# volume-em/empanada

Hardware: AMD Instinct MI355X
Metric: Mvox/s end-to-end 3D panoptic inference (incl. consensus); PQ vs CPU ref (higher is better)
Workload: dtype f32

## Files before the change

empanada_amd/_hip.py:

```python
import ctypes
import os

import torch

_HERE = os.path.dirname(os.path.abspath(__file__))
LIB_PATH = os.path.join(_HERE, 'libemp_hip.so')

MAX_KS = 11
MAX_CLASSES = 16
MAX_CENTERS = 4096
CENTER_LIMIT = 65535


class HipError(RuntimeError):
    pass


_c = ctypes
_P = _c.c_void_p
_I = _c.c_int
_L = _c.c_int64
_F = _c.c_float
_U32 = _c.c_uint32

SIGNATURES = {
    'emp_version': (_I, []),
    'emp_last_error': (_c.c_char_p, []),
    'emp_device_count': (_I, []),
    'emp_bn_act_nhwc': (_I, [_P, _P, _P, _P, _I, _L, _I, _P, _L, _P]),
    'emp_dwconv_nhwc': (_I, [_P, _P, _P, _I, _I, _I, _I, _I, _P, _P]),
    'emp_upsample_bilinear': (_I, [_P, _I, _I, _I, _I, _P, _P, _I, _I, _P, _P]),
    'emp_conv_bn_act_proj_nhwc': (_I, [_P, _P, _P, _P, _I] + [_I] * 10 + [_P, _I, _P, _P, _L, _P]),
    'emp_conv_k_slab': (_I, [_L, _I, _I, _I]),
    'emp_conv_k_slab_cin': (_I, [_L, _I, _I, _I, _I]),
    'emp_conv_k_slab_geom': (_I, [_L, _I, _I, _I, _I, _I, _I, _I, _I]),
    'emp_conv1x1_ws_eligible': (_I, [_L, _I, _I, _I, _I, _I, _I, _I]),
    'emp_conv1x1_ws_kind_for': (_I, [_L, _I, _I, _I, _I, _I, _I, _I, _I]),
    'emp_conv1x1_ws_launches': (_L, [_I]),
    'emp_gconv_chunk': (_I, [_I]),
    'emp_gconv3x3_bn_act_nhwc': (_I, [_P, _L, _P, _P, _P, _I, _I, _I, _I, _I, _I, _I, _P, _L, _P]),
    'emp_conv_bn_act_nhwc': (_I, [_P, _P, _P, _P, _P, _L, _I] + [_I] * 10 + [_P, _L, _P]),
    'emp_conv_splitk_plan': (_I, [_L, _I, _I, _I, _I]),
    'emp_conv_splitk_bn_act_nhwc': (_I, [_P, _P, _P, _P, _P, _L, _I] + [_I] * 11 + [_P, _P, _L, _P]),
    'emp_wino_input_transform': (_I, [_P, _I, _I, _I, _I, _I, _P, _L, _P, _P]),
    'emp_gemm_nt_batched': (_I, [_P, _P, _I, _L, _I, _I, _P, _P]),
    'emp_wino4_input_transform': (_I, [_P, _I, _I, _I, _I, _I, _P, _L, _P, _P]),
    'emp_wino4_output_transform': (_I, [_P, _P, _L, _I, _I, _I, _I, _I, _P, _P, _I, _P, _L, _P]),
    'emp_wino4_conv_bn_act_nhwc': (_I, [_P, _I, _I, _I, _I, _I, _P, _L, _P, _I, _P, _P, _I, _P, _L, _P]),
    'emp_wino4_fused_eligible': (_I, [_L, _I, _I, _I]),
    'emp_wino3_input_transform': (_I, [_P, _I, _I, _I, _I, _I, _P, _L, _P, _P]),
    'emp_wino3_output_transform': (_I, [_P, _P, _L, _I, _I, _I, _I, _I, _P, _P, _I, _P, _L, _P]),
    'emp_wino_gemm_fused': (_I, [_P, _I, _I, _I, _I, _I, _P, _L, _P, _I, _P, _P]),
    'emp_wino_output_transform': (_I, [_P, _P, _L, _I, _I, _I, _I, _I, _P, _P, _I, _P, _L, _P]),
    'emp_chain_class': (_I, [_L, _P, _P, _P, _I, _P, _P, _P, _P, _L, _L, _c.c_double, _c.c_double, _P, _P, _P, _P]),
    'emp_lsap_maximize': (_L, [_P, _L, _L, _P, _P]),
    'emp_slices_to_input': (_I, [_P, _L, _L, _L, _I, _I, _I, _I, _I, _F, _F, _P, _P]),
    'emp_slices_to_input_scaled': (_I, [_P, _L, _L, _L] + [_I] * 7 + [_P, _P, _P, _P, _I, _F, _F, _P, _P]),
    'emp_pointwise_out_nhwc': (_I, [_P, _P, _P, _L, _L, _I, _I, _P, _P]),
    'emp_bn_relu_maxpool_nhwc': (_I, [_P, _P, _P, _I, _I, _I, _I, _P, _P]),
    'emp_stem_conv7_bn_relu_maxpool': (_I, [_P, _P, _P, _P, _I, _I, _I, _P, _P]),
    'emp_logits_to_prob': (_I, [_P, _I, _I, _L, _P, _P]),
    'emp_upsample_bilinear_prob': (_I, [_P, _I, _I, _I, _I, _P, _P, _I, _I, _P, _I, _P]),
    'emp_pr_upsample2x': (_I, [_P, _I, _I, _I, _I, _P, _P, _P]),
    'emp_pr_topk_work_bytes': (_L, [_I, _L]),
    'emp_pr_topk': (_I, [_P, _I, _L, _I, _P, _L, _P, _P]),
    'emp_pr_point_sample': (_I, [_P, _L, _P, _I, _I, _I, _I, _I, _P, _I, _I, _I, _P, _P, _I, _P]),
    'emp_pr_scatter': (_I, [_P, _I, _P, _I, _I, _I, _L, _P, _P]),
    'emp_median_harden_stack': (_I, [_P, _I, _I, _L, _I, _F, _P, _P, _P]),
# ... 979 lines not shown
```

empanada_amd/csrc/emp_conv.hip:

```cpp
#include "emp_common.h"
#include "emp_wino4.h"
#include <stdlib.h>

typedef float f32x16 __attribute__((ext_vector_type(16)));

#define CG_BM 128
#define CG_BK 32
#define CG_THREADS 256

struct ConvGeom {
    const float *x, *w, *scale, *shift, *res;
    float *out;
    int N, H, W, Cin, OH, OW, Cout, KH, KW, stride, pad, dil, relu;
    int64_t M, out_ps, res_ps;
    int tiles_m, tiles_n;
    int64_t x_bs, w_bs, out_bs;
    const int32_t *tiles;
    const float *proj_w;
    float *proj_out;
    int proj_n;
    int64_t hw;
};

__device__ __attribute__((aligned(16))) float cg_zero_page[64];

__device__ __forceinline__ void cg_glds16(const float *src, unsigned lds_byte_addr)
{
    asm volatile("s_mov_b32 m0, %1\n\ts_nop 0\n\tglobal_load_lds_dwordx4 %0, off" ::"v"(src), "s"(lds_byte_addr) : "memory", "m0");
}

template <int N>
__device__ __forceinline__ void cg_wait_vm()
{
    asm volatile("s_waitcnt vmcnt(%0)" ::"n"(N) : "memory");
}

template <int NT, int MODE, bool RESPF = false, int BK = 32, bool PROJ = false, bool GLDS = false, bool GATE = false>
__global__ __launch_bounds__(CG_THREADS, (BK == 16 ? 3 : 2)) void conv_igemm_f32_kernel(ConvGeom g)
{
    constexpr int BN = 64 * NT;
    constexpr int CG_LD = GLDS ? BK : BK + 4;
    constexpr int NBUF = GLDS ? (BK == 16 ? 3 : 2) : 2;
    constexpr int TPR = BK / 4;
    constexpr int RPP = CG_THREADS / TPR;
    constexpr int AR = CG_BM / RPP;
    constexpr int BROWS = BN / RPP;
    constexpr int NF4 = BK / 8;
    constexpr int CLD = BN + 4;
    constexpr int A_ELEMS = NBUF * CG_BM * CG_LD, B_ELEMS = NBUF * BN * CG_LD;
    constexpr int EPI_ROWS = (A_ELEMS + B_ELEMS >= CG_BM * CLD) ? CG_BM : 64;
    constexpr int C_ELEMS = EPI_ROWS * CLD;
    constexpr int SMEM = (A_ELEMS + B_ELEMS) > C_ELEMS ? (A_ELEMS + B_ELEMS) : C_ELEMS;
    static_assert(MODE == 0 || BK == 32, "the fused Winograd loader is written for BK = 32");
    static_assert(!GLDS || MODE == 0, "LDS-direct staging: plain convolution / GEMM loader only");
    __shared__ __attribute__((aligned(16))) float smem[SMEM];
    float *As = smem, *Bs = smem + A_ELEMS;
    g.x += (int64_t)blockIdx.y * g.x_bs;
    g.w += (int64_t)blockIdx.y * g.w_bs;
    g.out += (int64_t)blockIdx.y * g.out_bs;

    const int T = g.tiles_m * g.tiles_n;
    const int chunk = (T + 7) >> 3;
    const int tile = (blockIdx.x & 7) * chunk + (blockIdx.x >> 3);
    if (tile >= T) return;
    const int tm = tile / g.tiles_n, tn = tile % g.tiles_n;
    const int64_t m0 = (int64_t)tm * CG_BM;
    const int n0 = tn * BN;

    const int tid = threadIdx.x;
    const int lrow = tid / TPR, lcol = (tid % TPR) * 4;

    int a_n[AR], a_iy[AR], a_ix[AR];
    bool a_ok[AR], b_ok[BROWS];
    const float *b_ptr[BROWS];
    const int taps = g.KH * g.KW;
    int w_off[4][4];
    unsigned w_mask[4];
    float w_su = 1.f, w_sv = 1.f;
    if constexpr (MODE == 0) {
#pragma unroll
        for (int i = 0; i < AR; ++i) {
            const int64_t p = m0 + lrow + RPP * i;
            a_ok[i] = p < g.M;
            const int64_t pp = a_ok[i] ? p : 0;
            const int ox = (int)(pp % g.OW);
            const int oy = (int)((pp / g.OW) % g.OH);
            a_n[i] = (int)(pp / ((int64_t)g.OW * g.OH));
// ... 133 lines not shown
        for (int it = 0; it < NRE; ++it) {
            const int64_t p = m0 + crow + it * RPI;
            rpre[it] = make_float4(0.f, 0.f, 0.f, 0.f);
            if (p < g.M && co + 3 < g.Cout) rpre[it] = *reinterpret_cast<const float4 *>(g.res + p * g.res_ps + co);
        }
    }

    if constexpr (GLDS) {
        constexpr int RPW = 64 / TPR;
        constexpr int NL = AR + BROWS;
        const int swz_ld = (BK == 16) ? ((lrow >> 2) & 3) : ((lrow >> 1) & 7);
        const int csw = (((tid % TPR) ^ swz_ld) * 4);
        const float *ga[AR], *gb[BROWS];
        bool ga_ok[AR];
        auto set_tap_g = [&](int tap) {
            const int ky = tap / g.KW, kx = tap - ky * g.KW;
#pragma unroll
            for (int i = 0; i < AR; ++i) {
                const int iy = a_iy[i] + ky * g.dil, ix = a_ix[i] + kx * g.dil;
                ga_ok[i] = a_ok[i] && iy >= 0 && iy < g.H && ix >= 0 && ix < g.W;
                ga[i] = ga_ok[i] ? g.x + (((int64_t)a_n[i] * g.H + iy) * g.W + ix) * g.Cin + csw : cg_zero_page + csw;
            }
        };
#pragma unroll
        for (int i = 0; i < BROWS; ++i) {
            const int cob = n0 + lrow + RPP * i;
            gb[i] = (cob < g.Cout) ? g.w + (int64_t)cob * taps * g.Cin + csw : cg_zero_page + csw;
        }
        set_tap_g(tap0);
        const unsigned lds0 = (unsigned)(size_t)(__attribute__((address_space(3))) float *)smem;
        const unsigned a_dst = __builtin_amdgcn_readfirstlane(lds0 + (unsigned)(RPW * wave * BK * 4));
        const unsigned b_dst = __builtin_amdgcn_readfirstlane(lds0 + (unsigned)((A_ELEMS + RPW * wave * BK) * 4));
        int gl_tap = tap0, gl_c0 = c00;
        auto issue_slab = [&](int ring) {
#pragma unroll
            for (int i = 0; i < AR; ++i)
                cg_glds16(ga[i] + (ga_ok[i] ? gl_c0 : 0), a_dst + (unsigned)((ring * CG_BM + RPP * i) * BK * 4));
#pragma unroll
            for (int i = 0; i < BROWS; ++i) {
                const bool ok = n0 + lrow + RPP * i < g.Cout;
                cg_glds16(gb[i] + (ok ? (int64_t)gl_tap * g.Cin + gl_c0 : 0), b_dst + (unsigned)((ring * BN + RPP * i) * BK * 4));
            }
            gl_c0 += BK;
            if (gl_c0 == g.Cin) {
                gl_c0 = 0;
                ++gl_tap;
                if (gl_tap < taps) set_tap_g(gl_tap);
            }
        };
        const int swz_rd = (BK == 16) ? ((r >> 2) & 3) : ((r >> 1) & 7);
        issue_slab(0);
        if (NBUF == 3 && S > 1) issue_slab(1);
        if (NBUF == 3 && S > 1) cg_wait_vm<NL>(); else cg_wait_vm<0>();
        __builtin_amdgcn_s_barrier();
        for (int s = 0; s < S; ++s) {
            const int ring = s % NBUF;
            if (s + NBUF - 1 < S) issue_slab((s + NBUF - 1) % NBUF);
            const float *Ar = &As[ring * CG_BM * CG_LD + (wm * 64 + r) * CG_LD];
            const float *Br = &Bs[ring * BN * CG_LD + (wn * 32 * NT + r) * CG_LD];
#pragma unroll
            for (int f = 0; f < NF4; ++f) {
                const int pc = (((hh * NF4 + f) ^ swz_rd) * 4);
                float4 fa[2], fb[NT];
#pragma unroll
                for (int i = 0; i < 2; ++i) fa[i] = *reinterpret_cast<const float4 *>(Ar + i * 32 * CG_LD + pc);
#pragma unroll
                for (int j = 0; j < NT; ++j) fb[j] = *reinterpret_cast<const float4 *>(Br + j * 32 * CG_LD + pc);
#pragma unroll
                for (int e = 0; e < 4; ++e) {
                    float av[2], bv[NT];
#pragma unroll
                    for (int i = 0; i < 2; ++i) av[i] = e == 0 ? fa[i].x : e == 1 ? fa[i].y : e == 2 ? fa[i].z : fa[i].w;
#pragma unroll
                    for (int j = 0; j < NT; ++j) bv[j] = e == 0 ? fb[j].x : e == 1 ? fb[j].y : e == 2 ? fb[j].z : fb[j].w;
#pragma unroll
                    for (int i = 0; i < 2; ++i)
#pragma unroll
                        for (int j = 0; j < NT; ++j)
                            acc[i][j] = __builtin_amdgcn_mfma_f32_32x32x2f32(av[i], bv[j], acc[i][j], 0, 0, 0);
                }
            }
            if (NBUF == 3 && s + 2 < S) cg_wait_vm<NL>(); else cg_wait_vm<0>();
            __builtin_amdgcn_s_barrier();
        }
    } else {
        CG_LOAD_NEXT();
        store_slab(0);
        if (S > 1) CG_LOAD_NEXT();
        __syncthreads();
        for (int s = 0; s < S; ++s) {
            const int buf = s & 1;
            const float *Ab = &As[buf * CG_BM * CG_LD + (wm * 64 + r) * CG_LD + hh * (BK / 2)];
            const float *Bb = &Bs[buf * BN * CG_LD + (wn * 32 * NT + r) * CG_LD + hh * (BK / 2)];
    #pragma unroll
            for (int half = 0; half < NF4 / 2; ++half) {
                float4 fa[2][2], fb[NT][2];
    #pragma unroll
                for (int q = 0; q < 2; ++q) {
    #pragma unroll
                    for (int i = 0; i < 2; ++i)
                        fa[i][q] = *reinterpret_cast<const float4 *>(Ab + i * 32 * CG_LD + half * 8 + q * 4);
    #pragma unroll
                    for (int j = 0; j < NT; ++j)
                        fb[j][q] = *reinterpret_cast<const float4 *>(Bb + j * 32 * CG_LD + half * 8 + q * 4);
                }
    #pragma unroll
                for (int q = 0; q < 2; ++q) {
    #pragma unroll
                    for (int e = 0; e < 4; ++e) {
                        float av[2], bv[NT];
    #pragma unroll
                        for (int i = 0; i < 2; ++i)
                            av[i] = e == 0 ? fa[i][q].x : e == 1 ? fa[i][q].y : e == 2 ? fa[i][q].z : fa[i][q].w;
    #pragma unroll
                        for (int j = 0; j < NT; ++j)
// ... 106 lines not shown
            if constexpr (PROJ) {
                float ps[4] = {0.f, 0.f, 0.f, 0.f};
                if (valid && co + 3 < g.Cout) {
#pragma unroll
                    for (int q = 0; q < 4; ++q)
                        if (q < g.proj_n) {
                            const float4 wq = *reinterpret_cast<const float4 *>(g.proj_w + (int64_t)q * g.Cout + co);
                            ps[q] = __fadd_rn(__fadd_rn(__fadd_rn(__fmul_rn(v[0], wq.x), __fmul_rn(v[1], wq.y)),
                                                        __fmul_rn(v[2], wq.z)), __fmul_rn(v[3], wq.w));
                        }
                }
                *reinterpret_cast<float4 *>(&Cs[lrow_c * CLD + ccol]) = make_float4(ps[0], ps[1], ps[2], ps[3]);
            }
        }
        if constexpr (PROJ) {
            __syncthreads();
            for (int idx = tid; idx < EPI_ROWS * g.proj_n; idx += CG_THREADS) {
                const int row_l = idx / g.proj_n, q = idx - row_l * g.proj_n;
                const int64_t p = m0 + rd * EPI_ROWS + row_l;
                if (p < g.M) {
                    float t = Cs[row_l * CLD + q];
#pragma unroll 8
                    for (int j = 1; j < C4; ++j) t = __fadd_rn(t, Cs[row_l * CLD + 4 * j + q]);
                    const int64_t img = p / g.hw;
                    atomicAdd(g.proj_out + (img * g.proj_n + q) * g.hw + (p - img * g.hw), t);
                }
            }
        }
    }
}

struct CgPlan {
    bool narrow, respf, glds;
    int slab, tiles_m, tiles_n;
};

static CgPlan cg_plan(int64_t M, int Cout, int batch, bool has_res, bool res_vec_ok, bool may_split_n = true, int cin = 32)
{
    CgPlan p;
    const int64_t wide_blocks = emp_cdiv(M, CG_BM) * emp_cdiv(Cout, 128) * batch;
    p.narrow = Cout <= 64 || (Cout % 128 != 0 && Cout % 128 <= 64 && Cout < 512) || (may_split_n && wide_blocks < 256);
    p.tiles_m = (int)emp_cdiv(M, CG_BM);
    p.tiles_n = (int)emp_cdiv(Cout, p.narrow ? 64 : 128);
    static const char *fnarrow = getenv("EMP_CONV_NARROW");
    static const char *norespf = getenv("EMP_CONV_NO_RESPF");
    if (fnarrow && fnarrow[0] == '1') {
        p.narrow = true;
        p.tiles_n = (int)emp_cdiv(Cout, 64);
    }
    p.respf = has_res && res_vec_ok && Cout % (p.narrow ? 64 : 128) == 0 && !norespf;
    static const char *force = getenv("EMP_CONV_BK");
    const int64_t blocks = (int64_t)p.tiles_m * p.tiles_n * batch;
    p.slab = blocks > 512 ? 16 : 32;
    if (force && force[0] == '1') p.slab = 16;
    if (force && force[0] == '3') p.slab = 32;
    if (p.respf) p.slab = 32;
    if (cin % 32 != 0) {
        p.slab = 16;
        p.respf = false;
    }
    static const char *noglds = getenv("EMP_CONV_NO_GLDS");
    p.glds = !noglds;
    return p;
}

extern "C" int emp_conv_k_slab(int64_t M, int Cout, int batch, int has_residual)
{
    return cg_plan(M, Cout, batch, has_residual != 0, true).slab;
}

extern "C" int emp_conv_k_slab_cin(int64_t M, int Cout, int batch, int has_residual, int Cin)
{
    return cg_plan(M, Cout, batch, has_residual != 0, true, true, Cin).slab;
}

extern "C" __attribute__((visibility("hidden"))) int emp_conv1x1_ws_kind(int64_t M, int Cin, int Cout, int KH, int KW, int stride, int pad, int relu, int has_residual);
extern "C" __attribute__((visibility("hidden"))) int emp_conv1x1_ws_launch(int kind, const float *x, const float *w, const float *scale, const float *shift,
                                     const float *res, int64_t res_ps, int relu, int64_t M, int Cin, int Cout,
                                     float *out, int64_t out_ps, void *stream);
extern "C" __attribute__((visibility("hidden"))) int emp_gemm_ws_eligible(int batch, int64_t M, int N, int K, int slab);
extern "C" __attribute__((visibility("hidden"))) int emp_gemm_ws_launch(const float *A, const float *B, int batch, int64_t M, int N, int K, float *C,
                                                                        void *stream);

extern "C" int emp_conv_k_slab_geom(int64_t M, int Cout, int has_residual, int Cin, int KH, int KW, int stride, int pad,
                                    int relu)
{
    if (emp_conv1x1_ws_kind(M, Cin, Cout, KH, KW, stride, pad, relu, has_residual) == 1) return 64;
    return cg_plan(M, Cout, 1, has_residual != 0 && relu != 2, true, true, Cin).slab;
}

extern "C" int emp_conv_bn_act_nhwc(const float *x, const float *w_okkc, const float *scale, const float *shift,
                                    const float *residual, int64_t res_pixel_stride, int relu, int N, int H, int W,
                                    int Cin, int Cout, int KH, int KW, int stride, int pad, int dil, float *out,
                                    int64_t out_pixel_stride, void *stream)
{
// ... 12 lines not shown
                "conv: x and w must be 16-byte aligned");
    EMP_REQUIRE(out != x, "conv: output cannot alias the input");
    if (N == 0) return EMP_OK;
    ConvGeom g;
    g.x = x; g.w = w_okkc; g.scale = scale; g.shift = shift; g.res = residual; g.out = out;
    g.N = N; g.H = H; g.W = W; g.Cin = Cin; g.OH = OH; g.OW = OW; g.Cout = Cout; g.KH = KH; g.KW = KW;
    g.stride = stride; g.pad = pad; g.dil = dil; g.relu = relu;
    g.M = (int64_t)N * OH * OW; g.out_ps = out_pixel_stride; g.res_ps = res_pixel_stride;
    g.x_bs = g.w_bs = g.out_bs = 0; g.tiles = nullptr; g.proj_w = nullptr; g.proj_out = nullptr; g.proj_n = 0; g.hw = 1;
    const bool res_vec_ok = (res_pixel_stride & 3) == 0 && (reinterpret_cast<uintptr_t>(residual) & 15) == 0;
    const bool io_vec_ok = res_vec_ok && (out_pixel_stride & 3) == 0 && (reinterpret_cast<uintptr_t>(out) & 15) == 0 &&
                           (!scale || (reinterpret_cast<uintptr_t>(scale) & 15) == 0) &&
                           (!shift || (reinterpret_cast<uintptr_t>(shift) & 15) == 0);
    const int ws = io_vec_ok && scale && shift ? emp_conv1x1_ws_kind(g.M, Cin, Cout, KH, KW, stride, pad, relu, residual != nullptr) : 0;
    if (ws == 1)
        return emp_conv1x1_ws_launch(1, x, w_okkc, scale, shift, residual, res_pixel_stride, relu, g.M, Cin, Cout, out,
                                     out_pixel_stride, stream);
    const CgPlan pl = cg_plan(g.M, Cout, 1, residual != nullptr && relu != 2, res_vec_ok, true, Cin);
    if (ws == 2 && !residual && pl.slab == 16)
        return emp_conv1x1_ws_launch(2, x, w_okkc, scale, shift, nullptr, res_pixel_stride, relu, g.M, Cin, Cout, out,
                                     out_pixel_stride, stream);
    if (ws == 3 && residual && pl.respf && pl.slab == 32 &&
        res_pixel_stride < (1 << 24) && out_pixel_stride < (1 << 24))
        return emp_conv1x1_ws_launch(3, x, w_okkc, scale, shift, residual, res_pixel_stride, relu, g.M, Cin, Cout, out,
                                     out_pixel_stride, stream);
    const bool narrow = pl.narrow, respf = pl.respf, bk16 = pl.slab == 16;
    EMP_REQUIRE((int64_t)pl.tiles_m * pl.tiles_n < (1LL << 28), "conv: too many tiles");
    g.tiles_m = pl.tiles_m;
    g.tiles_n = pl.tiles_n;
    const int T = g.tiles_m * g.tiles_n;
    const int grid = 8 * ((T + 7) / 8);
#define CG_GO(NT_, RES_, BK_, GL_) hipLaunchKernelGGL((conv_igemm_f32_kernel<NT_, 0, RES_, BK_, false, GL_>), dim3(grid), dim3(CG_THREADS), 0, emp_stream(stream), g)
#define CG_GATE(NT_, BK_) hipLaunchKernelGGL((conv_igemm_f32_kernel<NT_, 0, false, BK_, false, true, true>), dim3(grid), dim3(CG_THREADS), 0, emp_stream(stream), g)
    if (relu == 2) {
        if (narrow) { if (bk16) CG_GATE(1, 16); else CG_GATE(1, 32); }
        else { if (bk16) CG_GATE(2, 16); else CG_GATE(2, 32); }
    } else if (narrow) {
        if (respf) { if (pl.glds) CG_GO(1, true, 32, true); else CG_GO(1, true, 32, false); }
        else if (pl.glds) { if (bk16) CG_GO(1, false, 16, true); else CG_GO(1, false, 32, true); }
        else { if (bk16) CG_GO(1, false, 16, false); else CG_GO(1, false, 32, false); }
    } else {
        if (respf) { if (pl.glds) CG_GO(2, true, 32, true); else CG_GO(2, true, 32, false); }
        else if (pl.glds) { if (bk16) CG_GO(2, false, 16, true); else CG_GO(2, false, 32, true); }
        else { if (bk16) CG_GO(2, false, 16, false); else CG_GO(2, false, 32, false); }
    }
#undef CG_GO
#undef CG_GATE
    EMP_CHECK_LAUNCH("emp_conv_bn_act_nhwc");
    return EMP_OK;
}

__global__ __launch_bounds__(256) void splitk_reduce_kernel(const float *__restrict__ work, int nz, int64_t M, int Cout,
                                                            const float *__restrict__ scale,
                                                            const float *__restrict__ shift,
                                                            const float *__restrict__ res, int64_t res_ps, int relu,
                                                            float *__restrict__ out, int64_t out_ps)
{
    const int C4 = Cout >> 2;
    const int64_t total = M * C4, plane = M * (int64_t)Cout;
    for (int64_t i = (int64_t)blockIdx.x * blockDim.x + threadIdx.x; i < total; i += (int64_t)gridDim.x * blockDim.x) {
        const int64_t p = i / C4;
        const int co = (int)(i - p * C4) * 4;
        const float *w = work + p * Cout + co;
        float4 t = *reinterpret_cast<const float4 *>(w);
        for (int z = 1; z < nz; ++z) {
            const float4 u = *reinterpret_cast<const float4 *>(w + z * plane);
            t.x = __fadd_rn(t.x, u.x); t.y = __fadd_rn(t.y, u.y); t.z = __fadd_rn(t.z, u.z); t.w = __fadd_rn(t.w, u.w);
        }
        float v[4] = {t.x, t.y, t.z, t.w};
#pragma unroll
        for (int e = 0; e < 4; ++e) {
            const float sc = scale ? scale[co + e] : 1.f, sh = shift ? shift[co + e] : 0.f;
            v[e] = __fadd_rn(__fmul_rn(v[e], sc), sh);
        }
        if (res) {
            const float4 r4 = *reinterpret_cast<const float4 *>(res + p * res_ps + co);
// ... 45 lines not shown
    EMP_REQUIRE(out != x && work != x && work != out, "conv_splitk: buffers must not alias");
    if (N == 0) return EMP_OK;
    ConvGeom g;
    g.x = x; g.w = w_okkc; g.scale = nullptr; g.shift = nullptr; g.res = nullptr; g.out = work;
    g.N = N; g.H = H; g.W = W; g.Cin = Cin; g.OH = OH; g.OW = OW; g.Cout = Cout; g.KH = KH; g.KW = KW;
    g.stride = stride; g.pad = pad; g.dil = dil; g.relu = 0;
    g.M = (int64_t)N * OH * OW; g.out_ps = Cout; g.res_ps = Cout;
    g.x_bs = g.w_bs = g.out_bs = 0; g.tiles = nullptr; g.proj_w = nullptr; g.proj_out = nullptr; g.proj_n = 0; g.hw = 1;
    const CgPlan pl = cg_plan(g.M, Cout, 1, false, true, true, Cin);
    EMP_REQUIRE((int64_t)pl.tiles_m * pl.tiles_n < (1LL << 28), "conv_splitk: too many tiles");
    g.tiles_m = pl.tiles_m;
    g.tiles_n = pl.tiles_n;
    const int T = g.tiles_m * g.tiles_n;
    const dim3 grid(8 * ((T + 7) / 8), 1, k_splits);
    hipStream_t st = emp_stream(stream);
    if (pl.narrow)
        hipLaunchKernelGGL((conv_igemm_f32_kernel<1, 0, false, 32, false, true>), grid, dim3(CG_THREADS), 0, st, g);
    else
        hipLaunchKernelGGL((conv_igemm_f32_kernel<2, 0, false, 32, false, true>), grid, dim3(CG_THREADS), 0, st, g);
    EMP_CHECK_LAUNCH("emp_conv_splitk_bn_act_nhwc(partials)");
    const int64_t total = g.M * (Cout / 4);
    hipLaunchKernelGGL(splitk_reduce_kernel, dim3(emp_grid(total, 256, 4096)), dim3(256), 0, st, work, k_splits, g.M, Cout,
                       scale, shift, residual, res_pixel_stride, relu, out, out_pixel_stride);
    EMP_CHECK_LAUNCH("emp_conv_splitk_bn_act_nhwc(reduce)");
    return EMP_OK;
}

extern "C" int emp_conv_bn_act_proj_nhwc(const float *x, const float *w_okkc, const float *scale, const float *shift,
                                         int relu, int N, int H, int W, int Cin, int Cout, int KH, int KW, int stride,
                                         int pad, int dil, const float *proj_w, int proj_n, float *proj_out,
                                         float *out, int64_t out_pixel_stride, void *stream)
{
    EMP_REQUIRE(x && w_okkc && proj_w && proj_out, "conv_proj: null pointer");
    EMP_REQUIRE(N >= 0 && H > 0 && W > 0 && Cin > 0 && Cin % CG_BK == 0, "conv_proj: bad shape (Cin %% %d)", CG_BK);
    EMP_REQUIRE(Cout == 128 || Cout == 256, "conv_proj: Cout %d must be 128 or 256 (at most two cout tiles)", Cout);
    EMP_REQUIRE(proj_n >= 1 && proj_n <= 4, "conv_proj: proj_n %d not in 1..4", proj_n);
    EMP_REQUIRE(KH >= 1 && KW >= 1 && KH <= 7 && KW <= 7 && stride >= 1 && dil >= 1 && pad >= 0, "conv_proj: bad filter geometry");
    const int OH = (H + 2 * pad - dil * (KH - 1) - 1) / stride + 1;
    const int OW = (W + 2 * pad - dil * (KW - 1) - 1) / stride + 1;
    EMP_REQUIRE(OH > 0 && OW > 0, "conv_proj: empty output");
    if (out_pixel_stride == 0) out_pixel_stride = Cout;
    EMP_REQUIRE(((reinterpret_cast<uintptr_t>(x) | reinterpret_cast<uintptr_t>(w_okkc) | reinterpret_cast<uintptr_t>(proj_w) |
                  reinterpret_cast<uintptr_t>(out)) & 15) == 0 && (out_pixel_stride & 3) == 0, "conv_proj: alignment");
    EMP_REQUIRE(out != x, "conv_proj: output cannot alias the input");
    if (N == 0) return EMP_OK;
    ConvGeom g;
    g.x = x; g.w = w_okkc; g.scale = scale; g.shift = shift; g.res = nullptr; g.out = out;
    g.N = N; g.H = H; g.W = W; g.Cin = Cin; g.OH = OH; g.OW = OW; g.Cout = Cout; g.KH = KH; g.KW = KW;
    g.stride = stride; g.pad = pad; g.dil = dil; g.relu = relu;
    g.M = (int64_t)N * OH * OW; g.out_ps = out_pixel_stride; g.res_ps = Cout;
    g.x_bs = g.w_bs = g.out_bs = 0; g.tiles = nullptr;
    g.proj_w = proj_w; g.proj_out = proj_out; g.proj_n = proj_n; g.hw = (int64_t)OH * OW;
    const CgPlan pl = cg_plan(g.M, Cout, 1, false, true, false);
    g.tiles_m = pl.tiles_m;
    g.tiles_n = pl.tiles_n;
    const int T = g.tiles_m * g.tiles_n;
    const int grid = 8 * ((T + 7) / 8);
#define CG_GOP(BK_, GL_) hipLaunchKernelGGL((conv_igemm_f32_kernel<2, 0, false, BK_, true, GL_>), dim3(grid), dim3(CG_THREADS), 0, emp_stream(stream), g)
    if (pl.glds) { if (pl.slab == 16) CG_GOP(16, true); else CG_GOP(32, true); }
    else { if (pl.slab == 16) CG_GOP(16, false); else CG_GOP(32, false); }
#undef CG_GOP
    EMP_CHECK_LAUNCH("emp_conv_bn_act_proj_nhwc");
    return EMP_OK;
}


__global__ __launch_bounds__(256) void wino_input_kernel(const float *__restrict__ x, const int32_t *__restrict__ tiles,
                                                         int64_t T, int H, int W, int C4, int dil, float4 *__restrict__ V)
{
    const int64_t total = T * C4;
    for (int64_t i = (int64_t)blockIdx.x * blockDim.x + threadIdx.x; i < total; i += (int64_t)gridDim.x * blockDim.x) {
        const int c4 = (int)(i % C4);
        const int64_t t = i / C4;
        const int n = tiles[3 * t], by = tiles[3 * t + 1], bx = tiles[3 * t + 2];
        const float4 *src = reinterpret_cast<const float4 *>(x) + (int64_t)n * H * W * C4 + c4;
        float4 d[4][4];
#pragma unroll
        for (int a = 0; a < 4; ++a)
#pragma unroll
            for (int b = 0; b < 4; ++b) {
                const int yy = by + a * dil, xx = bx + b * dil;
                d[a][b] = make_float4(0.f, 0.f, 0.f, 0.f);
                if (yy >= 0 && yy < H && xx >= 0 && xx < W) d[a][b] = src[((int64_t)yy * W + xx) * C4];
            }
#define W_SUB(p, q) make_float4(__fsub_rn(p.x, q.x), __fsub_rn(p.y, q.y), __fsub_rn(p.z, q.z), __fsub_rn(p.w, q.w))
#define W_ADD(p, q) make_float4(__fadd_rn(p.x, q.x), __fadd_rn(p.y, q.y), __fadd_rn(p.z, q.z), __fadd_rn(p.w, q.w))
        float4 tt[4][4];
#pragma unroll
        for (int a = 0; a < 4; ++a) {
            tt[a][0] = W_SUB(d[a][0], d[a][2]);
            tt[a][1] = W_ADD(d[a][1], d[a][2]);
            tt[a][2] = W_SUB(d[a][2], d[a][1]);
// ... 46 lines not shown
            for (int b = 0; b < 2; ++b) {
                const int yy = oy + a * dil, xx = ox + b * dil;
                if (yy < H && xx < W) {
                    float4 v = yv[b];
                    if (scale) v = make_float4(__fmul_rn(v.x, sc.x), __fmul_rn(v.y, sc.y), __fmul_rn(v.z, sc.z), __fmul_rn(v.w, sc.w));
                    if (shift) v = W_ADD(v, sh);
                    if (relu) v = make_float4(fmaxf(v.x, 0.f), fmaxf(v.y, 0.f), fmaxf(v.z, 0.f), fmaxf(v.w, 0.f));
                    *reinterpret_cast<float4 *>(out + (((int64_t)n * H + yy) * W + xx) * out_ps + 4 * c4) = v;
                }
            }
        }
    }
}
#undef W_SUB
#undef W_ADD

extern "C" int emp_wino_input_transform(const float *x, int N, int H, int W, int C, int dil, const int32_t *tiles,
                                        int64_t T, float *V, void *stream)
{
    EMP_REQUIRE(x && tiles && V, "wino_input: null pointer");
    EMP_REQUIRE(N > 0 && H > 0 && W > 0 && C > 0 && C % 4 == 0 && dil >= 1 && T >= 0, "wino_input: bad shape");
    EMP_REQUIRE(((reinterpret_cast<uintptr_t>(x) | reinterpret_cast<uintptr_t>(V)) & 15) == 0, "wino_input: alignment");
    if (T == 0) return EMP_OK;
    hipLaunchKernelGGL(wino_input_kernel, dim3(emp_grid(T * (C / 4), 256, 16384)), dim3(256), 0, emp_stream(stream), x,
                       tiles, T, H, W, C / 4, dil, reinterpret_cast<float4 *>(V));
    EMP_CHECK_LAUNCH("emp_wino_input_transform");
    return EMP_OK;
}

extern "C" int emp_gemm_nt_batched(const float *A, const float *B, int batch, int64_t M, int N, int K, float *C,
                                   void *stream)
{
    EMP_REQUIRE(A && B && C, "gemm: null pointer");
    EMP_REQUIRE(batch >= 1 && batch <= 65535 && M >= 0 && M < (1LL << 31) && N > 0 && K > 0 && K % CG_BK == 0,
                "gemm: bad shape (K must be a multiple of %d)", CG_BK);
    EMP_REQUIRE(((reinterpret_cast<uintptr_t>(A) | reinterpret_cast<uintptr_t>(B)) & 15) == 0, "gemm: alignment");
    if (M == 0) return EMP_OK;
    ConvGeom g;
    g.x = A; g.w = B; g.scale = g.shift = g.res = nullptr; g.out = C;
    g.N = 1; g.H = 1; g.W = (int)M; g.Cin = K; g.OH = 1; g.OW = (int)M; g.Cout = N; g.KH = g.KW = 1;
    g.stride = 1; g.pad = 0; g.dil = 1; g.relu = 0;
    g.M = M; g.out_ps = N; g.res_ps = N;
    g.x_bs = M * K; g.w_bs = (int64_t)N * K; g.out_bs = M * N; g.tiles = nullptr; g.proj_w = nullptr; g.proj_out = nullptr; g.proj_n = 0; g.hw = 1;
    const CgPlan pl = cg_plan(M, N, batch, false, true);
    if ((reinterpret_cast<uintptr_t>(C) & 15) == 0 && emp_gemm_ws_eligible(batch, M, N, K, pl.slab))
        return emp_gemm_ws_launch(A, B, batch, M, N, K, C, stream);
    const bool narrow = pl.narrow, bk16 = pl.slab == 16;
    g.tiles_m = pl.tiles_m;
    g.tiles_n = pl.tiles_n;
    const int T = g.tiles_m * g.tiles_n;
    dim3 grid(8 * ((T + 7) / 8), batch);
#define CG_GOG(NT_, BK_, GL_) hipLaunchKernelGGL((conv_igemm_f32_kernel<NT_, 0, false, BK_, false, GL_>), grid, dim3(CG_THREADS), 0, emp_stream(stream), g)
    if (narrow) {
        if (pl.glds) { if (bk16) CG_GOG(1, 16, true); else CG_GOG(1, 32, true); }
        else { if (bk16) CG_GOG(1, 16, false); else CG_GOG(1, 32, false); }
    } else {
        if (pl.glds) { if (bk16) CG_GOG(2, 16, true); else CG_GOG(2, 32, true); }
        else { if (bk16) CG_GOG(2, 16, false); else CG_GOG(2, 32, false); }
    }
#undef CG_GOG
    EMP_CHECK_LAUNCH("emp_gemm_nt_batched");
    return EMP_OK;
}

extern "C" int emp_wino_gemm_fused(const float *x, int N, int H, int W, int Cin, int dil, const int32_t *tiles,
                                   int64_t T, const float *U, int Cout, float *Mw, void *stream)
{
    EMP_REQUIRE(x && tiles && U && Mw, "wino_gemm: null pointer");
    EMP_REQUIRE(N > 0 && H > 0 && W > 0 && Cin > 0 && Cin % CG_BK == 0 && Cout > 0 && dil >= 1 && T >= 0,
                "wino_gemm: bad shape (Cin must be a multiple of %d)", CG_BK);
    EMP_REQUIRE((int64_t)N * H * W * Cin < (1LL << 31) && T < (1LL << 31), "wino_gemm: activation too large for 32-bit offsets");
    EMP_REQUIRE(((reinterpret_cast<uintptr_t>(x) | reinterpret_cast<uintptr_t>(U)) & 15) == 0, "wino_gemm: alignment");
    if (T == 0) return EMP_OK;
    ConvGeom g;
    g.x = x; g.w = U; g.scale = g.shift = g.res = nullptr; g.out = Mw;
    g.N = N; g.H = H; g.W = W; g.Cin = Cin; g.OH = 1; g.OW = 1; g.Cout = Cout; g.KH = g.KW = 1;
    g.stride = 1; g.pad = 0; g.dil = dil; g.relu = 0;
    g.M = T; g.out_ps = Cout; g.res_ps = Cout;
    g.x_bs = 0; g.w_bs = (int64_t)Cout * Cin; g.out_bs = T * Cout; g.tiles = tiles; g.proj_w = nullptr; g.proj_out = nullptr; g.proj_n = 0; g.hw = 1;
    const bool narrow = Cout <= 64;
    g.tiles_m = (int)emp_cdiv(T, CG_BM);
    g.tiles_n = (int)emp_cdiv(Cout, narrow ? 64 : 128);
    const int nt = g.tiles_m * g.tiles_n;
    dim3 grid(8 * ((nt + 7) / 8), 16);
    if (narrow) hipLaunchKernelGGL((conv_igemm_f32_kernel<1, 1>), grid, dim3(CG_THREADS), 0, emp_stream(stream), g);
    else hipLaunchKernelGGL((conv_igemm_f32_kernel<2, 1>), grid, dim3(CG_THREADS), 0, emp_stream(stream), g);
    EMP_CHECK_LAUNCH("emp_wino_gemm_fused");
    return EMP_OK;
}

// ... 275 lines not shown
```

include/emp_hip.h:

```cpp
#ifndef EMP_HIP_H
#define EMP_HIP_H

#include <stdint.h>

#ifdef __cplusplus
extern "C" {
#endif

#define EMP_OK 0
#define EMP_EINVAL (-1)
#define EMP_ELAUNCH (-2)
#define EMP_ENODEV (-3)

#define EMP_MAX_KS 11
#define EMP_MAX_CLASSES 16
#define EMP_MAX_CENTERS 4096
#define EMP_CENTER_LIMIT 65535

int emp_version(void);
const char *emp_last_error(void);
int emp_device_count(void);

int emp_slices_to_input(const uint8_t *vol, int64_t stride_slice, int64_t stride_row, int64_t stride_col,
                        int n_slices, int h, int w, int hp, int wp, float mean255, float inv_std255,
                        float *out, void *stream);

int emp_slices_to_input_scaled(const uint8_t *vol, int64_t stride_slice, int64_t stride_row, int64_t stride_col,
                               int n_slices, int h, int w, int dh, int dw, int hp, int wp, const int32_t *row_off,
                               const int16_t *row_coef, const int32_t *col_off, const int16_t *col_coef, int area,
                               float mean255, float inv_std255, float *out, void *stream);

int emp_bn_act_nhwc(const float *x, const float *scale, const float *shift, const float *residual,
                    int relu, int64_t n_pixels, int C, float *out, int64_t out_pixel_stride, void *stream);

int emp_dwconv_nhwc(const float *x, const float *w_kkc, const float *bias, int N, int H, int W, int C,
                    int k, float *y, void *stream);

int emp_upsample_bilinear(const float *x, int N, int C, int h, int w, const int64_t *x_strides,
                          float *y, int H, int W, const int64_t *y_strides, void *stream);

int emp_conv_k_slab(int64_t M, int Cout, int batch, int has_residual);
int emp_conv_k_slab_cin(int64_t M, int Cout, int batch, int has_residual, int Cin);
int emp_conv_k_slab_geom(int64_t M, int Cout, int has_residual, int Cin, int KH, int KW, int stride, int pad, int relu);
int emp_conv1x1_ws_eligible(int64_t M, int Cin, int Cout, int KH, int KW, int stride, int pad, int relu);
int emp_conv1x1_ws_kind_for(int64_t M, int Cin, int Cout, int KH, int KW, int stride, int pad, int relu, int has_residual);
int64_t emp_conv1x1_ws_launches(int kind);
int emp_conv_bn_act_nhwc(const float *x, const float *w_okkc, const float *scale, const float *shift,
                         const float *residual, int64_t res_pixel_stride, int relu, int N, int H, int W,
                         int Cin, int Cout, int KH, int KW, int stride, int pad, int dil, float *out,
                         int64_t out_pixel_stride, void *stream);
int emp_conv_splitk_plan(int64_t M, int Cout, int Cin, int KH, int KW);
int emp_conv_splitk_bn_act_nhwc(const float *x, const float *w_okkc, const float *scale, const float *shift,
                                const float *residual, int64_t res_pixel_stride, int relu, int N, int H, int W,
                                int Cin, int Cout, int KH, int KW, int stride, int pad, int dil, int k_splits,
                                float *work, float *out, int64_t out_pixel_stride, void *stream);

int emp_conv_bn_act_proj_nhwc(const float *x, const float *w_okkc, const float *scale, const float *shift,
                              int relu, int N, int H, int W, int Cin, int Cout, int KH, int KW, int stride,
                              int pad, int dil, const float *proj_w, int proj_n, float *proj_out,
                              float *out, int64_t out_pixel_stride, void *stream);

int emp_gconv_chunk(int group_w);
int emp_gconv3x3_bn_act_nhwc(const float *x, int64_t x_pixel_stride, const float *w_okkc, const float *scale,
                             const float *shift, int relu, int N, int H, int W, int groups, int group_w,
                             int stride, float *out, int64_t out_pixel_stride, void *stream);

int emp_wino_input_transform(const float *x, int N, int H, int W, int C, int dil, const int32_t *tiles,
                             int64_t T, float *V, void *stream);
int emp_gemm_nt_batched(const float *A, const float *B, int batch, int64_t M, int N, int K, float *C,
                        void *stream);
int emp_wino_gemm_fused(const float *x, int N, int H, int W, int Cin, int dil, const int32_t *tiles,
                        int64_t T, const float *U, int Cout, float *Mw, void *stream);
int emp_wino_output_transform(const float *Mw, const int32_t *tiles, int64_t T, int N, int H, int W,
                              int Cout, int dil, const float *scale, const float *shift, int relu,
                              float *out, int64_t out_pixel_stride, void *stream);
// ... 167 lines not shown
```

Before: 133.8.

## Add configurable LDS ring depths for BK16 LDS-direct conv and use 2/2 for proj

Splits the A and B LDS staging rings of the BK=16 LDS-direct implicit-GEMM conv so each can hold two or three buffers, with a 3/2 variant that prefetches A two slabs ahead and B one ahead. Shallower rings shrink LDS per block and raise the launch-bounds occupancy target to four blocks. The projection-fused conv defaults to the 2/2 ring on large grids, and an env/API switch allows forcing a layout. The trade is less prefetch depth for more resident blocks. The GEMM and conv_proj paths now pass K/Cin to the planner and accept multiples of 16.

Measured after the change: 134.4, median of 3. No clear change (+0.5%).

```diff
diff --git a/empanada_amd/_hip.py b/empanada_amd/_hip.py
--- a/empanada_amd/_hip.py
+++ b/empanada_amd/_hip.py
@@ -34,6 +34,7 @@
     'emp_conv_k_slab': (_I, [_L, _I, _I, _I]),
     'emp_conv_k_slab_cin': (_I, [_L, _I, _I, _I, _I]),
     'emp_conv_k_slab_geom': (_I, [_L, _I, _I, _I, _I, _I, _I, _I, _I]),
+    'emp_conv_ring_layout': (_I, [_I]),
     'emp_conv1x1_ws_eligible': (_I, [_L, _I, _I, _I, _I, _I, _I, _I]),
     'emp_conv1x1_ws_kind_for': (_I, [_L, _I, _I, _I, _I, _I, _I, _I, _I]),
     'emp_conv1x1_ws_launches': (_L, [_I]),
diff --git a/empanada_amd/csrc/emp_conv.hip b/empanada_amd/csrc/emp_conv.hip
--- a/empanada_amd/csrc/emp_conv.hip
+++ b/empanada_amd/csrc/emp_conv.hip
@@ -35,24 +35,38 @@
     asm volatile("s_waitcnt vmcnt(%0)" ::"n"(N) : "memory");
 }
 
-template <int NT, int MODE, bool RESPF = false, int BK = 32, bool PROJ = false, bool GLDS = false, bool GATE = false>
-__global__ __launch_bounds__(CG_THREADS, (BK == 16 ? 3 : 2)) void conv_igemm_f32_kernel(ConvGeom g)
+#define CG_RING_33 0
+#define CG_RING_32 1
+#define CG_RING_22 2
+constexpr int cg_ring_a(int bk, bool glds, int ring) { return (glds && bk == 16 && ring != CG_RING_22) ? 3 : 2; }
+constexpr int cg_ring_b(int bk, bool glds, int ring) { return (glds && bk == 16 && ring == CG_RING_33) ? 3 : 2; }
+constexpr int cg_bound(int nt, int bk, bool glds, int ring)
+{
+    return bk != 16 ? 2 : (glds && (ring != CG_RING_33 || nt == 1)) ? 4 : 3;
+}
+
+template <int NT, int MODE, bool RESPF = false, int BK = 32, bool PROJ = false, bool GLDS = false, bool GATE = false,
+          int RING = CG_RING_33>
+__global__ __launch_bounds__(CG_THREADS, cg_bound(NT, BK, GLDS, RING)) void conv_igemm_f32_kernel(ConvGeom g)
 {
     constexpr int BN = 64 * NT;
     constexpr int CG_LD = GLDS ? BK : BK + 4;
-    constexpr int NBUF = GLDS ? (BK == 16 ? 3 : 2) : 2;
+    constexpr int NBA = cg_ring_a(BK, GLDS, RING), NBB = cg_ring_b(BK, GLDS, RING);
+    static_assert(RING == CG_RING_33 || (GLDS && BK == 16 && MODE == 0 && !RESPF), "ring layouts: LDS-direct BK = 16 only");
+    static_assert(RING != CG_RING_32 || NT == 2, "3/2: 128-wide cout tiles only");
     constexpr int TPR = BK / 4;
     constexpr int RPP = CG_THREADS / TPR;
     constexpr int AR = CG_BM / RPP;
     constexpr int BROWS = BN / RPP;
     constexpr int NF4 = BK / 8;
     constexpr int CLD = BN + 4;
-    constexpr int A_ELEMS = NBUF * CG_BM * CG_LD, B_ELEMS = NBUF * BN * CG_LD;
+    constexpr int A_ELEMS = NBA * CG_BM * CG_LD, B_ELEMS = NBB * BN * CG_LD;
     constexpr int EPI_ROWS = (A_ELEMS + B_ELEMS >= CG_BM * CLD) ? CG_BM : 64;
     constexpr int C_ELEMS = EPI_ROWS * CLD;
     constexpr int SMEM = (A_ELEMS + B_ELEMS) > C_ELEMS ? (A_ELEMS + B_ELEMS) : C_ELEMS;
     static_assert(MODE == 0 || BK == 32, "the fused Winograd loader is written for BK = 32");
     static_assert(!GLDS || MODE == 0, "LDS-direct staging: plain convolution / GEMM loader only");
+    static_assert(cg_bound(NT, BK, GLDS, RING) != 4 || SMEM * sizeof(float) <= 40960, "bound 4: at most 40 KiB of LDS per block");
     __shared__ __attribute__((aligned(16))) float smem[SMEM];
     float *As = smem, *Bs = smem + A_ELEMS;
     g.x += (int64_t)blockIdx.y * g.x_bs;
@@ -252,15 +266,20 @@
         const unsigned a_dst = __builtin_amdgcn_readfirstlane(lds0 + (unsigned)(RPW * wave * BK * 4));
         const unsigned b_dst = __builtin_amdgcn_readfirstlane(lds0 + (unsigned)((A_ELEMS + RPW * wave * BK) * 4));
         int gl_tap = tap0, gl_c0 = c00;
-        auto issue_slab = [&](int ring) {
+        int gb_tap = tap0, gb_c0 = c00;
+        auto issue_a = [&](int ring) {
 #pragma unroll
             for (int i = 0; i < AR; ++i)
                 cg_glds16(ga[i] + (ga_ok[i] ? gl_c0 : 0), a_dst + (unsigned)((ring * CG_BM + RPP * i) * BK * 4));
+        };
+        auto issue_b = [&](int ring, int tap, int c0) {
 #pragma unroll
             for (int i = 0; i < BROWS; ++i) {
                 const bool ok = n0 + lrow + RPP * i < g.Cout;
-                cg_glds16(gb[i] + (ok ? (int64_t)gl_tap * g.Cin + gl_c0 : 0), b_dst + (unsigned)((ring * BN + RPP * i) * BK * 4));
-            }
+                cg_glds16(gb[i] + (ok ? (int64_t)tap * g.Cin + c0 : 0), b_dst + (unsigned)((ring * BN + RPP * i) * BK * 4));
+            }
+        };
+        auto next_a = [&]() {
             gl_c0 += BK;
             if (gl_c0 == g.Cin) {
                 gl_c0 = 0;
@@ -268,16 +287,50 @@
                 if (gl_tap < taps) set_tap_g(gl_tap);
             }
         };
+        auto next_b = [&]() {
+            gb_c0 += BK;
+            if (gb_c0 == g.Cin) {
+                gb_c0 = 0;
+                ++gb_tap;
+            }
+        };
+        auto issue_slab = [&](int ring) {
+            issue_a(ring);
+            issue_b(ring, gl_tap, gl_c0);
+            next_a();
+        };
         const int swz_rd = (BK == 16) ? ((r >> 2) & 3) : ((r >> 1) & 7);
-        issue_slab(0);
-        if (NBUF == 3 && S > 1) issue_slab(1);
-        if (NBUF == 3 && S > 1) cg_wait_vm<NL>(); else cg_wait_vm<0>();
+        if constexpr (NBA == NBB) {
+            issue_slab(0);
+            if (NBA == 3 && S > 1) issue_slab(1);
+            if (NBA == 3 && S > 1) cg_wait_vm<NL>(); else cg_wait_vm<0>();
+        } else {
+            issue_a(0);
+            next_a();
+            issue_b(0, gb_tap, gb_c0);
+            next_b();
+            if (S > 1) {
+                issue_a(1);
+                next_a();
+                cg_wait_vm<AR>();
+            } else cg_wait_vm<0>();
+        }
         __builtin_amdgcn_s_barrier();
         for (int s = 0; s < S; ++s) {
-            const int ring = s % NBUF;
-            if (s + NBUF - 1 < S) issue_slab((s + NBUF - 1) % NBUF);
-            const float *Ar = &As[ring * CG_BM * CG_LD + (wm * 64 + r) * CG_LD];
-            const float *Br = &Bs[ring * BN * CG_LD + (wn * 32 * NT + r) * CG_LD];
+            if constexpr (NBA == NBB) {
+                if (s + NBA - 1 < S) issue_slab((s + NBA - 1) % NBA);
+            } else {
+                if (s + 1 < S) {
+                    issue_b((s + 1) % NBB, gb_tap, gb_c0);
+                    next_b();
+                }
+                if (s + 2 < S) {
+                    issue_a((s + 2) % NBA);
+                    next_a();
+                }
+            }
+            const float *Ar = &As[(s % NBA) * CG_BM * CG_LD + (wm * 64 + r) * CG_LD];
+            const float *Br = &Bs[(s % NBB) * BN * CG_LD + (wn * 32 * NT + r) * CG_LD];
 #pragma unroll
             for (int f = 0; f < NF4; ++f) {
                 const int pc = (((hh * NF4 + f) ^ swz_rd) * 4);
@@ -300,7 +353,11 @@
                             acc[i][j] = __builtin_amdgcn_mfma_f32_32x32x2f32(av[i], bv[j], acc[i][j], 0, 0, 0);
                 }
             }
-            if (NBUF == 3 && s + 2 < S) cg_wait_vm<NL>(); else cg_wait_vm<0>();
+            if constexpr (NBA == NBB) {
+                if (NBA == 3 && s + 2 < S) cg_wait_vm<NL>(); else cg_wait_vm<0>();
+            } else {
+                if (s + 2 < S) cg_wait_vm<AR>(); else cg_wait_vm<0>();
+            }
             __builtin_amdgcn_s_barrier();
         }
     } else {
@@ -473,10 +530,49 @@
 
 struct CgPlan {
     bool narrow, respf, glds;
-    int slab, tiles_m, tiles_n;
+    int slab, tiles_m, tiles_n, ring;
 };
 
-static CgPlan cg_plan(int64_t M, int Cout, int batch, bool has_res, bool res_vec_ok, bool may_split_n = true, int cin = 32)
+#define CG_RING_PROJ CG_RING_22
+#define CG_RING_WIDE CG_RING_33
+#define CG_RING_NARROW CG_RING_33
+
+static int cg_ring_force = -2;
+
+static int cg_ring_forced()
+{
+    if (cg_ring_force == -2) {
+        const char *e = getenv("EMP_CONV_RING");
+        cg_ring_force = !e ? -1 : (e[0] == '3' && e[1] == '3') ? CG_RING_33 : (e[0] == '3' && e[1] == '2') ? CG_RING_32 :
+                        (e[0] == '2' && e[1] == '2') ? CG_RING_22 : -1;
+    }
+    return cg_ring_force;
+}
+
+extern "C" int emp_conv_ring_layout(int set)
+{
+    const int was = cg_ring_forced();
+    cg_ring_force = (set == CG_RING_33 || set == CG_RING_32 || set == CG_RING_22) ? set : -1;
+    return was;
+}
+
+template <int NT, bool PROJ, bool GATE>
+static void cg_launch16(int ring, dim3 grid, hipStream_t st, const ConvGeom &g)
+{
+    if constexpr (NT == 2) {
+        if (ring == CG_RING_32) {
+            hipLaunchKernelGGL((conv_igemm_f32_kernel<2, 0, false, 16, PROJ, true, GATE, CG_RING_32>), grid, dim3(CG_THREADS), 0, st, g);
+            return;
+        }
+    }
+    if (ring == CG_RING_22)
+        hipLaunchKernelGGL((conv_igemm_f32_kernel<NT, 0, false, 16, PROJ, true, GATE, CG_RING_22>), grid, dim3(CG_THREADS), 0, st, g);
+    else
+        hipLaunchKernelGGL((conv_igemm_f32_kernel<NT, 0, false, 16, PROJ, true, GATE, CG_RING_33>), grid, dim3(CG_THREADS), 0, st, g);
+}
+
+static CgPlan cg_plan(int64_t M, int Cout, int batch, bool has_res, bool res_vec_ok, bool may_split_n = true, int cin = 32,
+                      bool proj = false)
 {
     CgPlan p;
     const int64_t wide_blocks = emp_cdiv(M, CG_BM) * emp_cdiv(Cout, 128) * batch;
@@ -502,6 +598,11 @@
     }
     static const char *noglds = getenv("EMP_CONV_NO_GLDS");
     p.glds = !noglds;
+    p.ring = CG_RING_33;
+    if (p.glds && p.slab == 16 && !p.respf) {
+        if (blocks > 512) p.ring = proj ? CG_RING_PROJ : p.narrow ? CG_RING_NARROW : CG_RING_WIDE;
+        if (cg_ring_forced() >= 0) p.ring = cg_ring_forced();
+    }
     return p;
 }
 
@@ -580,16 +681,17 @@
     const int grid = 8 * ((T + 7) / 8);
 #define CG_GO(NT_, RES_, BK_, GL_) hipLaunchKernelGGL((conv_igemm_f32_kernel<NT_, 0, RES_, BK_, false, GL_>), dim3(grid), dim3(CG_THREADS), 0, emp_stream(stream), g)
 #define CG_GATE(NT_, BK_) hipLaunchKernelGGL((conv_igemm_f32_kernel<NT_, 0, false, BK_, false, true, true>), dim3(grid), dim3(CG_THREADS), 0, emp_stream(stream), g)
+    const int ring = pl.ring;
     if (relu == 2) {
-        if (narrow) { if (bk16) CG_GATE(1, 16); else CG_GATE(1, 32); }
-        else { if (bk16) CG_GATE(2, 16); else CG_GATE(2, 32); }
+        if (narrow) { if (bk16) cg_launch16<1, false, true>(ring, dim3(grid), emp_stream(stream), g); else CG_GATE(1, 32); }
+        else { if (bk16) cg_launch16<2, false, true>(ring, dim3(grid), emp_stream(stream), g); else CG_GATE(2, 32); }
     } else if (narrow) {
         if (respf) { if (pl.glds) CG_GO(1, true, 32, true); else CG_GO(1, true, 32, false); }
-        else if (pl.glds) { if (bk16) CG_GO(1, false, 16, true); else CG_GO(1, false, 32, true); }
+        else if (pl.glds) { if (bk16) cg_launch16<1, false, false>(ring, dim3(grid), emp_stream(stream), g); else CG_GO(1, false, 32, true); }
         else { if (bk16) CG_GO(1, false, 16, false); else CG_GO(1, false, 32, false); }
     } else {
         if (respf) { if (pl.glds) CG_GO(2, true, 32, true); else CG_GO(2, true, 32, false); }
-        else if (pl.glds) { if (bk16) CG_GO(2, false, 16, true); else CG_GO(2, false, 32, true); }
+        else if (pl.glds) { if (bk16) cg_launch16<2, false, false>(ring, dim3(grid), emp_stream(stream), g); else CG_GO(2, false, 32, true); }
         else { if (bk16) CG_GO(2, false, 16, false); else CG_GO(2, false, 32, false); }
     }
 #undef CG_GO
@@ -701,7 +803,7 @@
                                          float *out, int64_t out_pixel_stride, void *stream)
 {
     EMP_REQUIRE(x && w_okkc && proj_w && proj_out, "conv_proj: null pointer");
-    EMP_REQUIRE(N >= 0 && H > 0 && W > 0 && Cin > 0 && Cin % CG_BK == 0, "conv_proj: bad shape (Cin %% %d)", CG_BK);
+    EMP_REQUIRE(N >= 0 && H > 0 && W > 0 && Cin > 0 && Cin % 16 == 0, "conv_proj: bad shape (Cin %% 16)");
     EMP_REQUIRE(Cout == 128 || Cout == 256, "conv_proj: Cout %d must be 128 or 256 (at most two cout tiles)", Cout);
     EMP_REQUIRE(proj_n >= 1 && proj_n <= 4, "conv_proj: proj_n %d not in 1..4", proj_n);
     EMP_REQUIRE(KH >= 1 && KW >= 1 && KH <= 7 && KW <= 7 && stride >= 1 && dil >= 1 && pad >= 0, "conv_proj: bad filter geometry");
@@ -720,13 +822,13 @@
     g.M = (int64_t)N * OH * OW; g.out_ps = out_pixel_stride; g.res_ps = Cout;
     g.x_bs = g.w_bs = g.out_bs = 0; g.tiles = nullptr;
     g.proj_w = proj_w; g.proj_out = proj_out; g.proj_n = proj_n; g.hw = (int64_t)OH * OW;
-    const CgPlan pl = cg_plan(g.M, Cout, 1, false, true, false);
+    const CgPlan pl = cg_plan(g.M, Cout, 1, false, true, false, Cin, true);
     g.tiles_m = pl.tiles_m;
     g.tiles_n = pl.tiles_n;
     const int T = g.tiles_m * g.tiles_n;
     const int grid = 8 * ((T + 7) / 8);
 #define CG_GOP(BK_, GL_) hipLaunchKernelGGL((conv_igemm_f32_kernel<2, 0, false, BK_, true, GL_>), dim3(grid), dim3(CG_THREADS), 0, emp_stream(stream), g)
-    if (pl.glds) { if (pl.slab == 16) CG_GOP(16, true); else CG_GOP(32, true); }
+    if (pl.glds) { if (pl.slab == 16) cg_launch16<2, true, false>(pl.ring, dim3(grid), emp_stream(stream), g); else CG_GOP(32, true); }
     else { if (pl.slab == 16) CG_GOP(16, false); else CG_GOP(32, false); }
 #undef CG_GOP
     EMP_CHECK_LAUNCH("emp_conv_bn_act_proj_nhwc");
@@ -839,8 +941,8 @@
                                    void *stream)
 {
     EMP_REQUIRE(A && B && C, "gemm: null pointer");
-    EMP_REQUIRE(batch >= 1 && batch <= 65535 && M >= 0 && M < (1LL << 31) && N > 0 && K > 0 && K % CG_BK == 0,
-                "gemm: bad shape (K must be a multiple of %d)", CG_BK);
+    EMP_REQUIRE(batch >= 1 && batch <= 65535 && M >= 0 && M < (1LL << 31) && N > 0 && K > 0 && K % 16 == 0,
+                "gemm: bad shape (K must be a multiple of 16)");
     EMP_REQUIRE(((reinterpret_cast<uintptr_t>(A) | reinterpret_cast<uintptr_t>(B)) & 15) == 0, "gemm: alignment");
     if (M == 0) return EMP_OK;
     ConvGeom g;
@@ -849,7 +951,7 @@
     g.stride = 1; g.pad = 0; g.dil = 1; g.relu = 0;
     g.M = M; g.out_ps = N; g.res_ps = N;
     g.x_bs = M * K; g.w_bs = (int64_t)N * K; g.out_bs = M * N; g.tiles = nullptr; g.proj_w = nullptr; g.proj_out = nullptr; g.proj_n = 0; g.hw = 1;
-    const CgPlan pl = cg_plan(M, N, batch, false, true);
+    const CgPlan pl = cg_plan(M, N, batch, false, true, true, K);
     if ((reinterpret_cast<uintptr_t>(C) & 15) == 0 && emp_gemm_ws_eligible(batch, M, N, K, pl.slab))
         return emp_gemm_ws_launch(A, B, batch, M, N, K, C, stream);
     const bool narrow = pl.narrow, bk16 = pl.slab == 16;
@@ -859,10 +961,10 @@
     dim3 grid(8 * ((T + 7) / 8), batch);
 #define CG_GOG(NT_, BK_, GL_) hipLaunchKernelGGL((conv_igemm_f32_kernel<NT_, 0, false, BK_, false, GL_>), grid, dim3(CG_THREADS), 0, emp_stream(stream), g)
     if (narrow) {
-        if (pl.glds) { if (bk16) CG_GOG(1, 16, true); else CG_GOG(1, 32, true); }
+        if (pl.glds) { if (bk16) cg_launch16<1, false, false>(pl.ring, grid, emp_stream(stream), g); else CG_GOG(1, 32, true); }
         else { if (bk16) CG_GOG(1, 16, false); else CG_GOG(1, 32, false); }
     } else {
-        if (pl.glds) { if (bk16) CG_GOG(2, 16, true); else CG_GOG(2, 32, true); }
+        if (pl.glds) { if (bk16) cg_launch16<2, false, false>(pl.ring, grid, emp_stream(stream), g); else CG_GOG(2, 32, true); }
         else { if (bk16) CG_GOG(2, 16, false); else CG_GOG(2, 32, false); }
     }
 #undef CG_GOG
diff --git a/include/emp_hip.h b/include/emp_hip.h
--- a/include/emp_hip.h
+++ b/include/emp_hip.h
@@ -41,6 +41,7 @@
 
 int emp_conv_k_slab(int64_t M, int Cout, int batch, int has_residual);
 int emp_conv_k_slab_cin(int64_t M, int Cout, int batch, int has_residual, int Cin);
+int emp_conv_ring_layout(int set);
 int emp_conv_k_slab_geom(int64_t M, int Cout, int has_residual, int Cin, int KH, int KW, int stride, int pad, int relu);
 int emp_conv1x1_ws_eligible(int64_t M, int Cin, int Cout, int KH, int KW, int stride, int pad, int relu);
 int emp_conv1x1_ws_kind_for(int64_t M, int Cin, int Cout, int KH, int KW, int stride, int pad, int relu, int has_residual);
```
